# ag14774/MPILattice-Boltzmann

Measured on AMD Instinct MI355X. Metric: MLUPS, higher is better.
Workload: dtype f32; 1 GPU; synthetic 8192x8192 D2Q9-BGK deck (walls + p=0.005 random obstacles, splitmix64 seed 42), density 0.1 accel 0.005 omega 1.85; nx=8192, ny=8192, partitioning=single GPU, loop=single, macro_k=0, launches_per_exchange=1, step_allreduce=False, kernel=lbm_multi_kernel<4>

## Files before the change

mpilattice-boltzmann_amd/csrc/kernels/multi.h:

```cpp
#pragma once
#include "common.h"

namespace {

#if LBM_TILE_STAMPS
#define LBM_MSTAMP(i) do { if (blockIdx.x == (gridDim.x >> 1) && threadIdx.x == 0) g_tile_stamps[i] = __builtin_amdgcn_s_memtime(); } while (0)
#else
#define LBM_MSTAMP(i) do { } while (0)
#endif

template <int K, int GEOM = kGeomStd>
struct MultiGeom {
  static constexpr int TX = geom_tx(GEOM);
  static constexpr int TY = multi_ty(K, GEOM);
  static constexpr int LANES = multi_lanes(K, GEOM);
  static constexpr int EY = K - 1, EX = multi_ex(K - 1);
  static constexpr int W = TX + 2 * EX, H = TY + 2 * EY;
  static constexpr int cells = W * H;
  static constexpr size_t lds_bytes = sizeof(float) * 9 * cells + sizeof(double) * K * (LANES / 64) + (K >= 2 ? cells / 2 : 0);
  static constexpr int blocks_per_cu = lds_bytes * 8 <= 160 * 1024 ? 8 : static_cast<int>(160 * 1024 / lds_bytes);
  static constexpr int waves_per_simd = blocks_per_cu * (LANES / 64) / 4 < LBM_MWAVES ? (blocks_per_cu * (LANES / 64) / 4 < 1 ? 1 : blocks_per_cu * (LANES / 64) / 4) : LBM_MWAVES;
  static constexpr bool owned_lanes = K == 4 && GEOM == kGeomTall;
  static constexpr int ring_pairs(int j) { return 2 * (K - j) * (TX / 2 + multi_ex(K - j)) + TY * multi_ex(K - j); }
};

struct MultiArgs {
  const float* src;
  float* dst;
  const float* srck[9];
  float* dstk[9];
  const uint32_t* mask;
  size_t ps;
  int nx;
  int row_first, rows_compute;
  int rows_storage;
  int count_first, count_end;
  int y_periodic;
  int y0_global, ny_global;
// ... 46 lines not shown
constexpr uint32_t kPairObstacles = 3u,
                   kPairKept = 4u,
                   kPairAccelRow = 8u,
                   kPairComputed = 16u,
                   kPairCounted = 32u;
__device__ __forceinline__ uint32_t pair_flag_bits(uint32_t mbits, bool kept, bool accel_row, bool counted)
{
  return mbits | (kept ? kPairKept : 0u) | (accel_row ? kPairAccelRow : 0u) | kPairComputed | (counted ? kPairCounted : 0u);
}

template <int K, int TERMS, int GEOM, int PART>
__global__ void __launch_bounds__((MultiGeom<K, GEOM>::LANES), (MultiGeom<K, GEOM>::waves_per_simd)) lbm_multi_kernel(const MultiArgs a)
{
  using G = MultiGeom<K, GEOM>;
  constexpr int TX = G::TX, EX = G::EX, EY = G::EY, W = G::W, WH = G::W / 2, kCells = G::cells, kLanes = G::LANES, kWaves = kLanes / 64, TY = G::TY;
  extern __shared__ __attribute__((aligned(16))) float lds[];
  double* red = reinterpret_cast<double*>(lds + 9 * kCells);
  uint8_t* pair_flags = reinterpret_cast<uint8_t*>(red + K * kWaves);
  const int tid = threadIdx.x;

  if (blockIdx.x == 0) {
    constexpr int kReadyWords = PART == kPartTile ? 4 : PART == kPartReady ? 2 : 0;
    if constexpr (kReadyWords > 0) {
      if (a.ready_epoch != 0ull && tid == 0) {
#pragma unroll
        for (int d = 0; d < kReadyWords; ++d) __hip_atomic_store(d < 2 ? a.ready[d] : a.ready_x[d - 2], a.ready_epoch, __ATOMIC_RELAXED, __HIP_MEMORY_SCOPE_SYSTEM);
      }
    }
    for (int v = 0; v < a.n_prev_vecs; ++v) {
      double s = 0.0;
      for (int i = tid; i < a.n_prev; i += kLanes) s += a.prev_partials[static_cast<size_t>(v) * a.n_prev + i];
      s = wave_sum(s);
// ... 111 lines not shown
  };
  auto classify = [&](auto count_c, const int fx, const int fy, const bool own, bool& kept, bool& counted) __attribute__((always_inline)) {
    constexpr bool COUNT = decltype(count_c)::value;
    const int srow = sy0 + fy - EY, gxo = x0 + fx - EX;
    kept = own;
    if (!inner) kept = kept && gxo < nx && srow < a.row_first + a.rows_compute;
    counted = COUNT ? (kept && srow >= a.count_first && srow < a.count_end) : kept;
    if constexpr (XR && COUNT) {
      kept = kept && gxo >= a.keep_x0 && gxo < a.keep_x1;
      counted = counted && kept && gxo >= a.cx0 && gxo < a.cx1;
    }
  };
  auto read_pair = [&](const int rd, const int fx, const int fy, f2 (&p)[9]) __attribute__((always_inline)) {
    const int ci = fy * W + fx - rd;
    const int cs = fy * W + (fx >> 1) - rd;
    p[2] = *reinterpret_cast<const f2*>(lds + 2 * kCells + ci - W);
    p[4] = *reinterpret_cast<const f2*>(lds + 4 * kCells + ci + W);
    p[1] = f2{lds[1 * kCells + cs - 1], lds[1 * kCells + cs + WH]};
    p[5] = f2{lds[5 * kCells + cs - W - 1], lds[5 * kCells + cs - W + WH]};
    p[8] = f2{lds[8 * kCells + cs + W - 1], lds[8 * kCells + cs + W + WH]};
    p[3] = f2{lds[3 * kCells + cs], lds[3 * kCells + cs + WH + 1]};
    p[6] = f2{lds[6 * kCells + cs - W], lds[6 * kCells + cs - W + WH + 1]};
    p[7] = f2{lds[7 * kCells + cs + W], lds[7 * kCells + cs + W + WH + 1]};
  };
  auto kept_cell = [&](const int fx, const int fy) __attribute__((always_inline)) { return tile_row_base + __mul24(fy - EY, nx) + x0 + fx - EX; };

  auto k_substeps = [&](auto count_c) __attribute__((always_inline)) {
    constexpr bool COUNT = decltype(count_c)::value;
    {
      const int ey = ksteps - 1, ex = multi_ex(ey);
      const int wp = (TX + 2 * ex) / 2;
      const int np = wp * (TY + 2 * ey);
  #pragma unroll 1
      for (int i = tid; i < np; i += kLanes) {
        const int ry = i / wp, rp = i - ry * wp;
        const int fx = EX - ex + 2 * rp, fy = EY - ey + ry;
        f2 p[9], out[9];
        uint32_t mbits = 0, o_here = 0;
// ... 74 lines not shown
    constexpr bool COUNT = decltype(count_c)::value;
    constexpr int TP = TX / 2;
    static_assert(TP * TY == kLanes && G::ring_pairs(1) <= kLanes, "one owned pair and at most one ring pair per lane and sub-step");
    auto ring_pos = [&](auto jc, const int i, int& fx, int& fy) __attribute__((always_inline)) {
      constexpr int ey = K - decltype(jc)::value, ex = multi_ex(ey), ep = ex / 2, wp = TP + ep * 2, band = ey * wp;
      if (i < 2 * band) {
        const bool top = i >= band;
        const int q = top ? i - band : i, ry = q / wp, rp = q - ry * wp;
        fy = top ? EY + TY + ry : EY - ey + ry;
        fx = EX - ex + 2 * rp;
      } else {
        const int q = i - 2 * band, ry = q / (2 * ep), c = q - ry * (2 * ep);
        fy = EY + ry;
        fx = EX - ex + 2 * (c < ep ? c : c + TP);
      }
    };
    auto relax = [&](const f2 (&p)[9], const uint32_t mbits, const bool accel, const uint32_t skip, f2 (&out)[9]) __attribute__((always_inline)) {
      const double term = finish_pair<TERMS>(p, mbits, a.omega, false, false, a.accel_w1, a.accel_w2, skip, out);
      if (tile_accel) accelerate_pair(out, mbits, accel, a.accel_w1, a.accel_w2);
      return term;
    };
    const int py = tid / TP, ofx = EX + 2 * (tid - py * TP), ofy = EY + py;
    f2 own0 = f2{0.0f, 0.0f};
    uint32_t ofl = 0;
    if (!COUNT && inner) {
      const float* const here0 = a.srck[0], * const here1 = a.srck[1] - 1, * const here3 = a.srck[3] + 1;
      const float* const south2 = a.srck[2] - nx, * const south5 = a.srck[5] - 1 - nx, * const south6 = a.srck[6] + 1 - nx;
      const float* const north4 = a.srck[4] + nx, * const north8 = a.srck[8] - 1 + nx, * const north7 = a.srck[7] + 1 + nx;
      typedef const __attribute__((address_space(1))) char* global_bytes;
      const uint32_t* mask_arg = a.mask;
// ... 9 lines not shown
        p[5] = at_byte<f2u>(south5, o);
        p[8] = at_byte<f2u>(north8, o);
        p[3] = at_byte<f2u>(here3, o);
        p[6] = at_byte<f2u>(south6, o);
        p[7] = at_byte<f2u>(north7, o);
        mbits = (*(const __attribute__((address_space(1))) uint32_t*)(mask + 4u * (static_cast<uint32_t>(cell) >> 5)) >> (cell & 31)) & 3u;
        return o;
      };
      {
        f2 p[9], out[9];
        uint32_t mbits;
        pull_inner(ofx, ofy, p, mbits);
        const bool accel_row_here = on_accel_row(sy0 + py);
        acc[0] = relax(p, mbits, accel_row_here, mbits, out);
  #pragma unroll
        for (int k = 1; k < 9; ++k) store_pair<W>(lds + k * kCells, k, ofy * W, ofx, out[k]);
        own0 = out[0];
        ofl = pair_flag_bits(mbits, true, accel_row_here, false);
      }
      if (tid < G::ring_pairs(1)) {
        int fx, fy;
        ring_pos(std::integral_constant<int, 1>{}, tid, fx, fy);
        f2 p[9], out[9];
        uint32_t mbits;
        pull_inner(fx, fy, p, mbits);
        const bool accel_row_here = on_accel_row(sy0 + fy - EY);
        relax(p, mbits, accel_row_here, 3u, out);
  #pragma unroll
        for (int k = 0; k < 9; ++k) store_pair<W>(lds + k * kCells, k, fy * W, fx, out[k]);
        pair_flags[(fy * W + fx) >> 1] = static_cast<uint8_t>(pair_flag_bits(mbits, false, accel_row_here, false));
      }
    } else {
  #pragma unroll 1
    for (int item = 0; item < 2; ++item) {
      const bool own = item == 0;
      if (!own && tid >= G::ring_pairs(1)) break;
      int fx = ofx, fy = ofy;
      if (!own) ring_pos(std::integral_constant<int, 1>{}, tid, fx, fy);
      f2 p[9];
      uint32_t mbits = 0, fl = 0, o_here = 0;
      int sr = 0;
      if (pull(fx, fy, p, mbits, sr, o_here)) {
        bool kept, counted;
        classify(count_c, fx, fy, own, kept, counted);
        const bool accel_row_here = on_accel_row(sr);
        f2 out[9];
        const double term = relax(p, mbits, accel_row_here, counted ? mbits : 3u, out);
  #pragma unroll
        for (int k = 1; k < 9; ++k) store_pair<W>(lds + k * kCells, k, fy * W, fx, out[k]);
        fl = pair_flag_bits(mbits, kept, accel_row_here, COUNT && counted);
        if (own) {
          acc[0] = term;
          own0 = out[0];
        } else {
          store_pair<W>(lds, 0, fy * W, fx, out[0]);
        }
      }
      if (own) ofl = fl;
      else pair_flags[(fy * W + fx) >> 1] = static_cast<uint8_t>(fl);
    }
    }
    LBM_MSTAMP(1);
    __syncthreads();
    LBM_MSTAMP(2);
    auto in_lds_substep = [&](auto jc) __attribute__((always_inline)) {
      constexpr int j = decltype(jc)::value;
      constexpr bool last = j == K;
      constexpr int rd = (j - 2) * W, wr = (j - 1) * W;
      f2 p[9], outs[9];
      read_pair(rd, ofx, ofy, p);
      p[0] = own0;
      const uint32_t mbits = ofl & kPairObstacles;
      const bool counted = (ofl & (COUNT ? kPairCounted : kPairKept)) != 0u;
      acc[j - 1] = relax(p, mbits, (!last || a.accel_last) && (ofl & kPairAccelRow), counted ? mbits : 3u, outs);
      own0 = outs[0];
      if constexpr (!last) {
        f2 q[9];
        int rfx = 0, rfy = 0;
        uint32_t rfl = 0;
        const bool ring = tid < G::ring_pairs(j);
        if (ring) {
          ring_pos(jc, tid, rfx, rfy);
          rfl = pair_flags[(rfy * W + rfx) >> 1];
          read_pair(rd, rfx, rfy, q);
          q[0] = *reinterpret_cast<const f2*>(lds + rfy * W + rfx - rd);
        }
        __syncthreads();
        if (ofl & kPairComputed) {
  #pragma unroll
          for (int k = 1; k < 9; ++k) store_pair<W>(lds + k * kCells, k, ofy * W - wr, ofx, outs[k]);
        }
        if (ring) {
          f2 routs[9];
          relax(q, rfl & kPairObstacles, (rfl & kPairAccelRow) != 0u, 3u, routs);
          if (rfl & kPairComputed) {
  #pragma unroll
            for (int k = 0; k < 9; ++k) store_pair<W>(lds + k * kCells, k, rfy * W - wr, rfx, routs[k]);
          }
        }
        __syncthreads();
      } else if (ofl & kPairKept) {
        const uint32_t o = 4u * static_cast<uint32_t>(kept_cell(ofx, ofy));
  #pragma unroll
        for (int k = 0; k < 9; ++k) __builtin_nontemporal_store(outs[k], &at_byte<f2>(a.dstk[k], o));
      }
      LBM_MSTAMP(1 + j);
    };
    in_lds_substep(std::integral_constant<int, 2>{});
    if constexpr (K >= 3) in_lds_substep(std::integral_constant<int, K >= 3 ? 3 : 2>{});
    if constexpr (K >= 4) in_lds_substep(std::integral_constant<int, K >= 4 ? 4 : 2>{});
  };
  auto substeps = [&](auto count_c) __attribute__((always_inline)) {
    if constexpr (G::owned_lanes) owned_substeps(count_c);
    else k_substeps(count_c);
  };

  if constexpr (PART == kPartGhost) {
    if (sy0 >= a.count_first && sy0 + TY <= a.count_end) substeps(std::false_type{});
    else substeps(std::true_type{});
  } else if constexpr (PART == kPartTile) {
    if (sy0 >= a.count_first && sy0 + TY <= a.count_end && x0 >= a.cx0 && x0 + TX <= a.cx1) substeps(std::false_type{});
    else substeps(std::true_type{});
  } else {
    substeps(std::false_type{});
  }

  if constexpr ((TERMS & ~kTermsFused) == kTermsCompensated && !G::owned_lanes) {
#pragma unroll
    for (int i = 0; i < K; ++i) acc[i] += static_cast<double>(acc_lo[i]);
  }
  if constexpr (K == 1) {
    const double w = wave_sum(acc[0]);
    if ((tid & 63) == 0) red[tid >> 6] = w;
  } else {
    static_assert(K <= 4, "wave_sum_vec4 carries four steps");
    const double w = wave_sum_vec4(acc[0], acc[1], K > 2 ? acc[2] : 0.0, K > 3 ? acc[K > 3 ? 3 : 0] : 0.0);
    const int q = wave_sum_slot<4>(tid & 63);
    if ((tid & 15) == 0 && q < K) red[q * kWaves + (tid >> 6)] = w;
  }
  lds_barrier();
  if (tid < ksteps) {
    double t = 0.0;
    for (int w = 0; w < kWaves; ++w) t += red[tid * kWaves + w];
    a.partials_out[static_cast<size_t>(tid) * a.ntiles_total + tile] = t;
  }
  LBM_MSTAMP(2 + K);
}

}
```

mpilattice-boltzmann_amd/csrc/lbm_geometry.h:

```cpp
#pragma once

namespace {

constexpr int kBlock = 256;
constexpr int kCellsPerLane = 4;
constexpr int kHaloGuard = 4;

constexpr int kTermsDouble = 0, kTermsFloat = 1, kTermsCompensated = 2, kTermsFused = 4;

constexpr int kMaxTileSteps = 8;

constexpr int kFoldSlices = 64;

constexpr int kPairCells = 2;

constexpr bool tile64_geom_ok(int t, int h) { return (t == 8 || t == 16) && (h == 4 || h == 8); }
constexpr int tile64_region(int t, int h) { return t + 2 * h; }
constexpr int tile64_block(int t, int h) { return (t == 8 && h == 4) ? 256 : 512; }
constexpr int tile64_lds_bytes(int t, int h)
{
  return tile64_region(t, h) * tile64_region(t, h) * (2 * 9 * 8 + 1) + 8 * h * (tile64_block(t, h) / 64);
}
constexpr int kTile64Rows = 4 * 2;
constexpr int tile64_row(int t, int h, bool full) { return ((t == 8 ? 2 : 0) + (h == 4 ? 1 : 0)) * 2 + (full ? 1 : 0); }
// ... 3 lines not shown
#define LBM_MTY 16
#define LBM_MLANES 512
#endif
#ifndef LBM_MWAVES
#define LBM_MWAVES 6
#endif
#ifndef LBM_MTY4
#define LBM_MTY4 13
#endif
#ifndef LBM_MTY4T
#define LBM_MTY4T 24
#define LBM_MLANES4T 768
#endif
constexpr int kMTX = 64, kMTXNarrow = 32, kMTY = LBM_MTY, kMTY4 = LBM_MTY4, kMTY4Tall = LBM_MTY4T, kMLanes = LBM_MLANES, kMLanes4Tall = LBM_MLANES4T,
              kMaxMultiSteps = 4,
              kMaxGhost = 32,
              kMaxGroup = 8;
constexpr int kMinMultiTY = kMTY < kMTY4 ? (kMTY < kMTY4Tall ? kMTY : kMTY4Tall) : (kMTY4 < kMTY4Tall ? kMTY4 : kMTY4Tall);
constexpr int kGeomStd = 0, kGeomNarrow = 1, kGeomTall = 2;
constexpr int geom_tx(int g) { return g == kGeomNarrow ? kMTXNarrow : kMTX; }
constexpr int multi_ty(int k, int g) { return k >= 4 ? (g == kGeomTall ? kMTY4Tall : kMTY4) : kMTY; }
constexpr int multi_lanes(int k, int g) { return (k >= 4 && g == kGeomTall) ? kMLanes4Tall : kMLanes; }
constexpr int geom_for(int k, int g) { return (g == kGeomTall && k < 4) ? kGeomStd : g; }

constexpr int multi_ex(int ey) { return 2 * ((ey + 1) / 2); }

constexpr int kMulti64TX = 32, kMulti64TY = 16, kMulti64Lanes = 512, kMulti64MinK = 2, kMulti64MaxK = 4;
constexpr int kMulti64Accs = 4;
constexpr bool multi64_k_ok(int k) { return k >= kMulti64MinK && k <= kMulti64MaxK; }
constexpr int multi64_frame_x(int k) { return kMulti64TX + 2 * multi_ex(k - 1); }
constexpr int multi64_frame_y(int k) { return kMulti64TY + 2 * (k - 1); }
constexpr int multi64_lds_bytes(int k)
{
  return multi64_frame_x(k) * multi64_frame_y(k) * (9 * 8 + 1) + 8 * kMulti64Accs * (kMulti64Lanes / 64);
}
constexpr int kMulti64Rows = (kMulti64MaxK - kMulti64MinK + 1) * 2 * 2;
constexpr int multi64_row(int k, bool nt, bool full) { return ((k - kMulti64MinK) * 2 + (nt ? 1 : 0)) * 2 + (full ? 1 : 0); }
static_assert(kMulti64TX * kMulti64TY == kMulti64Lanes, "the last sub-step deals one owned cell to every lane");
static_assert(kMulti64MaxK <= kMulti64Accs, "one accumulator per sub-step");
static_assert((kMulti64TX + 2 * (kMulti64MaxK - 2)) * (kMulti64TY + 2 * (kMulti64MaxK - 2)) <= 2 * kMulti64Lanes, "a frame sub-step deals a lane at most two cells");
static_assert(multi64_lds_bytes(kMulti64MaxK) <= 160 * 1024, "a block's LDS: at most what a CU gives one workgroup");

constexpr int kPartPlain = 0, kPartGhost = 1, kPartReady = 2, kPartTile = 3;

constexpr int kMultiTermsFused = 3;
constexpr int kMultiTerms = 4, kMultiParts = 4, kMultiGeoms = 3, kMultiRowsPerGeom = kMaxMultiSteps * kMultiTerms * kMultiParts;
constexpr int multi_row(int k, int geom, int terms, int part) { return ((geom * kMaxMultiSteps + k - 1) * kMultiTerms + terms) * kMultiParts + part; }
constexpr int kTileTermsFused = 2, kTileTerms = 3, kTileRows = 4 * 2 * kTileTerms;
constexpr int tile_row(int t, int h, bool full, int terms) { return (((t == 8 ? 2 : 0) + (h == 4 ? 1 : 0)) * 2 + (full ? 1 : 0)) * kTileTerms + terms; }

}
```

mpilattice-boltzmann_amd/csrc/lbm_internal.h:

```cpp
#pragma once
#include <cstddef>
#include <string>

#include "lbm_d2q9.h"
#include "lbm_d2q9_f64.h"
#include "lbm_knobs.h"

namespace lbm_internal {
void set_error(const std::string& msg);

struct ContextPlan {
  int nx, y0, nyl;
  unsigned flags;
  int self_periodic, accel_row;
  int use_graph;
  float accel_w1, accel_w2, free_cells_inv;
  int multi_K;
  int ghost;
  int ghost_rows;
  int group_max;
  int ghost_x, x0, nxl, nx_global, tiles_px, tiles_py, tile_rx, tile_ry;
  long long ncells, ncells_storage, ps, grid_floats;
  int mask_words, nxp;
  int nt_stores, lane_cells;
// ... 92 lines not shown
struct MacroRows { int bottom_edge_rows, interior_rows, top_edge_rows, left_cols, right_cols; };
MacroRows macro_rows(const ContextPlan& plan, int k, int ext);
bool edge_rows_suffice(const ContextPlan& plan, const GroupPlan& g, const MacroRows& rows, int next_total);
struct ColumnMessagePlan { int per, blocks; };
ColumnMessagePlan plan_column_message(const ContextPlan& plan, int cols, int max_blocks, const long long* peer, int npeer);
}

extern "C" int lbm_plan_next(int K, int four_rows, int tail4, int left);
extern "C" int lbm_plan_group_for(int K, int four_rows, int tail4, int ghost, int group_max, int left, int* steps, int cap);
extern "C" int lbm_plan_group(int K, int ghost, int group_max, int left, int* steps, int cap);
extern "C" int lbm_plan_sizeof(void);
extern "C" int lbm_plan_whole(const lbm_params* p, int free_cells, int y0, int ny_local, unsigned flags, int has_global_map, lbm_internal::ContextPlan* out);
extern "C" int lbm_plan_rank(const lbm_params* p, int free_cells, int nranks, int rank, unsigned flags, lbm_internal::ContextPlan* out);
extern "C" int lbm_plan_tile(const lbm_params* p, int free_cells, int px, int py, int rank, unsigned flags, lbm_internal::ContextPlan* out);
extern "C" int lbm_plan_kernel_name(const lbm_internal::ContextPlan* plan, char* kernel_name, size_t len);
extern "C" int lbm_plan_launch_sizeof(void);
extern "C" int lbm_plan_launch(const lbm_internal::ContextPlan* plan, int k, int ext, int which, int says_ready, lbm_internal::LaunchPlan* out);
extern "C" int lbm_plan_run_launches(const lbm_internal::ContextPlan* plan, int n_steps, int schedule, lbm_internal::LaunchPlan* out, int cap);
extern "C" int lbm_plan_edge_rows_suffice(const lbm_internal::ContextPlan* plan, int left);
extern "C" int lbm_plan64_sizeof(void);
extern "C" int lbm_plan64_whole(const lbm64_params* p, unsigned flags, lbm_internal::Plan64* out);
extern "C" int lbm_plan64_kernel_name(const lbm_internal::Plan64* plan, char* kernel_name, size_t len);
extern "C" int lbm_plan64_run_launches(const lbm_internal::Plan64* plan, int n_steps, int* steps, int* full, int cap);
extern "C" int lbm_plan64_multi_sizeof(void);
extern "C" int lbm_plan64_multi(const lbm64_params* p, unsigned flags, lbm_internal::PlanMulti64* out);
extern "C" int lbm_plan64_multi_kernel_name(const lbm_internal::PlanMulti64* plan, char* kernel_name, size_t len);
extern "C" int lbm_plan64_multi_run_launches(const lbm_internal::PlanMulti64* plan, int n_steps, int* steps, int* full, int cap);
extern "C" int lbm_plan64_rows_sizeof(void);
extern "C" int lbm_plan64_rows(const lbm64_params* p, int nranks, int rank, unsigned flags, lbm_internal::PlanRows64* out);
extern "C" int lbm_plan64_rows_kernel_name(const lbm_internal::PlanRows64* plan, char* kernel_name, size_t len);
// ... 1 lines not shown
```

mpilattice-boltzmann_amd/csrc/lbm_kernels.hip:

```cpp

#include <hip/hip_runtime.h>

#include <algorithm>
#include <array>
#include <cstdint>
#include <cstdio>
#include <cstdlib>
#include <cstring>
#include <string>
#include <thread>
#include <type_traits>
#include <utility>
#include <vector>

#include "lbm_d2q9.h"
#include "lbm_internal.h"
#include "lbm_knobs.h"
#include "kernels/common.h"
#include "kernels/step.h"
#include "kernels/tile.h"
#include "kernels/multi.h"
#include "kernels/aux.h"
#include "kernels/p2p.h"

// ... 151 lines not shown
{
  kStepKernels[c->plan.lane_cells == 1][c->plan.nt_stores][c->plan.fused]<<<dim3(blocks + 1), dim3(kBlock), 0, s>>>(a);
}

struct MultiKernel { void (*fn)(MultiArgs); size_t lds_bytes; };
static_assert(kTermsDouble == 0 && kTermsFloat == 1 && kTermsCompensated == 2 && kPartPlain == 0 && kPartTile == 3 && kGeomTall == 2, "the values index the table");
template <int ROW>
constexpr MultiKernel multi_kernel_row()
{
  constexpr int PART = ROW % kMultiParts, TERMS = ROW / kMultiParts % kMultiTerms, K = ROW / (kMultiParts * kMultiTerms) % kMaxMultiSteps + 1,
                GEOM = geom_for(K, ROW / kMultiRowsPerGeom);
  static_assert(multi_row(K, ROW / kMultiRowsPerGeom, TERMS, PART) == ROW, "multi_row and its inverse");
  static_assert(MultiGeom<K, GEOM>::LANES == multi_lanes(K, ROW / kMultiRowsPerGeom), "LaunchPlan::lanes is the row's block size");
  return {&lbm_multi_kernel<K, TERMS == kMultiTermsFused ? (kTermsCompensated | kTermsFused) : TERMS, GEOM, PART>, MultiGeom<K, GEOM>::lds_bytes};
}
template <size_t... ROW>
constexpr std::array<MultiKernel, sizeof...(ROW)> multi_kernel_rows(std::index_sequence<ROW...>) { return {{multi_kernel_row<static_cast<int>(ROW)>()...}}; }
constexpr auto kMultiKernels = multi_kernel_rows(std::make_index_sequence<kMultiGeoms * kMultiRowsPerGeom>{});

template <typename Table>
hipError_t raise_lds_limits(const Table& rows, int first, int end)
{
  for (int r = first; r < end; ++r) {
    if (rows[r].lds_bytes <= 65536) continue;
    const hipError_t e = hipFuncSetAttribute(reinterpret_cast<const void*>(rows[r].fn), hipFuncAttributeMaxDynamicSharedMemorySize, static_cast<int>(rows[r].lds_bytes));
    if (e != hipSuccess) return e;
  }
  return hipSuccess;
}
hipError_t raise_multi_lds_limits_for(int geom)
{
  return raise_lds_limits(kMultiKernels, geom * kMultiRowsPerGeom, (geom + 1) * kMultiRowsPerGeom);
}

using lbm_internal::LaunchPlan;
using lbm_internal::GroupPlan;
using lbm_internal::kLaunchWhole;
using lbm_internal::kLaunchInterior;
using lbm_internal::kLaunchEdge;

void launch_multi(lbm_ctx* c, const LaunchPlan& l, bool accel_last, bool fold, hipStream_t s)
{
  MultiArgs a{};
  a.src = c->grid[c->cur]; a.dst = c->grid[c->cur ^ 1];
  for (int k = 0; k < 9; ++k) { a.srck[k] = a.src + k * c->plan.ps; a.dstk[k] = a.dst + k * c->plan.ps; }
  a.mask = c->mask; a.ps = c->plan.ps; a.nx = c->p.nx;
  a.row_first = l.row_first; a.rows_compute = l.rows_compute; a.rows_storage = l.rows_storage;
// ... 245 lines not shown
  return 0;
}

static ColWindow col_window(const lbm_ctx* c) { return ColWindow{static_cast<unsigned>(c->p.nx), static_cast<unsigned>(c->plan.ghost_x), static_cast<unsigned>(c->plan.nxl)}; }
static size_t owned_cells(const lbm_ctx* c) { return static_cast<size_t>(c->plan.nxl) * c->plan.nyl; }

extern "C" {

int lbm_create(lbm_ctx** out, const lbm_params* p, int free_cells, const int* obstacles_rows, int y0,
               int ny_local, int device, unsigned flags)
{
  if (!out || !p || !obstacles_rows) { lbm_internal::set_error("lbm_create: null argument"); return 1; }
  *out = nullptr;
  const Knobs knobs = knobs_from_env();
  lbm_internal::ContextPlan plan;
  const int status = lbm_internal::plan_whole(knobs, p, free_cells, y0, ny_local, flags, false, &plan);
  return create_impl(out, status, plan, knobs, p, free_cells, obstacles_rows, nullptr, nullptr, device);
}

int lbm_create_global(lbm_ctx** out, const lbm_params* p, int free_cells, const int* obstacles_all, int y0,
                      int ny_local, int device, unsigned flags)
{
  if (!obstacles_all || !p || y0 < 0) { lbm_internal::set_error("lbm_create_global: bad argument"); return 1; }
  if (!out) { lbm_internal::set_error("lbm_create: null argument"); return 1; }
  *out = nullptr;
  const Knobs knobs = knobs_from_env();
  lbm_internal::ContextPlan plan;
  const int status = lbm_internal::plan_whole(knobs, p, free_cells, y0, ny_local, flags, true, &plan);
  return create_impl(out, status, plan, knobs, p, free_cells, obstacles_all + static_cast<size_t>(y0) * p->nx, obstacles_all, nullptr, device);
}

int lbm_create_rank(lbm_ctx** out, const lbm_params* p, int free_cells, const int* obstacle_window, int nranks,
                    int rank, int device, unsigned flags)
{
  if (!obstacle_window) { lbm_internal::set_error("lbm_create_rank: null argument"); return 1; }
  if (!out) {
    lbm_layout lay;
    if (lbm_rank_layout(p, nranks, rank, flags, &lay) == 0) lbm_internal::set_error("lbm_create: null argument");
    return 1;
  }
  *out = nullptr;
  const Knobs knobs = knobs_from_env();
  lbm_internal::ContextPlan plan;
// ... 591 lines not shown
```

mpilattice-boltzmann_amd/csrc/lbm_knobs.h:

```cpp
#pragma once

#include <climits>
#include <cstdlib>
#include <cstring>

constexpr int kKnobUnset = INT_MIN;
constexpr int kScheduleSerial = 0, kScheduleEdge = 1;

inline int schedule_of(const char* v) { return !std::strcmp(v, "serial") ? kScheduleSerial : !std::strcmp(v, "edge") ? kScheduleEdge : kKnobUnset; }
inline int knob_or(int v, int fallback) { return v == kKnobUnset ? fallback : v; }

#define LBM_KNOBS(X)                                                                        \
                                            \
  X(LBM_TUNE_SKEW,              skew,              24,         std::atoi)                   \
  X(LBM_TUNE_MAXBLOCKS,         maxblocks,         16384,      std::atoi)                   \
  X(LBM_TUNE_NARROW_MAX,        narrow_max,        65536,      std::atoi)                   \
  X(LBM_TUNE_TILE_MAX,          tile_max,          131072,     std::atoi)                   \
  X(LBM_TUNE_TILE_GEOM,         tile_geom,         kKnobUnset, std::atoi)                   \
  X(LBM_TUNE_TILE_SINGLE_MAX,   tile_single_max,   512,        std::atoi)                   \
  X(LBM_TUNE_TILE64_MAX,        tile64_max,        1 << 20,    std::atoi)                   \
  X(LBM_TUNE_TILE64_GEOM,       tile64_geom,       kKnobUnset, std::atoi)                   \
  X(LBM_TUNE_MULTI64_K,         multi64_k,         kKnobUnset, std::atoi)                   \
  X(LBM_TUNE_MULTI64_MIN,       multi64_min,       1 << 20,    std::atoi)                   \
  X(LBM_TUNE_MULTI_K,           multi_k,           kKnobUnset, std::atoi)                   \
  X(LBM_TUNE_MULTI_TAIL4,       multi_tail4,       1,          std::atoi)                   \
  X(LBM_TUNE_MULTI_TILE,        multi_tile,        kKnobUnset, std::atoi)                   \
  X(LBM_TUNE_NARROW_TILE_MAX,   narrow_tile_max,   1 << 17,    std::atoi)                   \
  X(LBM_TUNE_TALL_TILE_MIN,     tall_tile_min,     1 << 20,    std::atoi)                   \
  X(LBM_TUNE_MULTI_GEOM,        multi_geom,        -1,         std::atoi)                   \
  X(LBM_TUNE_MULTI_REMAP,       multi_remap,       1,          std::atoi)                   \
  X(LBM_TUNE_TILE_PAD_GRID,     tile_pad_grid,     1,          std::atoi)                   \
  X(LBM_TUNE_TERMS,             terms,             -1,         std::atoi)                   \
  X(LBM_TUNE_FOLD_SLICED_MIN,   fold_sliced_min,   1024,       std::atoi)                   \
  X(LBM_TUNE_OBS_CHUNK_CELLS,   obs_chunk_cells,   16 << 20,   std::atoi)                   \
  X(LBM_DEBUG_ADDR,             debug_addr,        0,          std::atoi)                   \
                    \
  X(LBM_TUNE_MACRO_K,           macro_k,           4,          std::atoi)                   \
  X(LBM_TUNE_MACRO_GHOST,       macro_ghost,       kKnobUnset, std::atoi)                   \
  X(LBM_TUNE_MACRO_GROUP,       macro_group,       kKnobUnset, std::atoi)                   \
// ... 27 lines not shown
```

mpilattice-boltzmann_amd/csrc/lbm_plan.cpp:

```cpp

#include <algorithm>
#include <cstdio>
#include <cstring>
#include <vector>

#include "lbm_d2q9.h"
#include "lbm_geometry.h"
#include "lbm_internal.h"
#include "lbm_knobs.h"

using lbm_internal::ContextPlan;
using lbm_internal::set_error;

namespace lbm_internal {

size_t plane_stride_floats(size_t ncells, int skew)
{
  size_t s = (ncells + 64 + 63) / 64 * 64;
  if ((s / 64) % 2 == 0) s += 64;
  if (ncells >= (1u << 20)) s += 64 * static_cast<size_t>(skew);
  return s;
}

int pick_iters(long long quads, int max_blocks)
// ... 112 lines not shown
  out->ghost_y = (py == 1 && !knobs.tile_ghost_rows) ? 0 : ghost;
  return 0;
}

struct TileSpec { int px, py, rx, ry, x0, nxl, ghost_x, nx_global, ghost_rows; };

void plan_multi(const Knobs& knobs, bool tile_rank, ContextPlan& c)
{
  c.multi_geom = pick_geom(knobs, static_cast<size_t>(c.ncells));
  if (tile_rank && c.ghost_rows == 0 && c.multi_geom == kGeomTall && knobs.multi_geom < 0) {
    auto over = [&](int ty) { return static_cast<double>((c.nyl + ty - 1) / ty * ty) / c.nyl; };
    if (over(kMTY4Tall) - over(kMTY4) > 0.03) c.multi_geom = kGeomStd;
  }
  c.multi_tx = geom_tx(c.multi_geom);
  c.multi_tiles_x = (c.nx + c.multi_tx - 1) / c.multi_tx;
  if (c.multi_K > 0) c.partials_cap = std::max(c.partials_cap, kMaxMultiSteps * c.multi_tiles_x * ((c.nyl + 2 * c.ghost_rows + kMinMultiTY - 1) / kMinMultiTY) + 1);
}

int plan_context(const Knobs& knobs, const lbm_params* p, int free_cells, bool has_global_map, bool has_window, int forced_k, int forced_ghost,
                 int y0, int ny_local, unsigned flags, const TileSpec* tile, ContextPlan* out)
{
  if (!p || !out) { set_error("lbm_create: null argument"); return lbm_internal::kPlanRefused; }
  if (p->nx < 1) { set_error("lbm_create: nx must be positive"); return lbm_internal::kPlanRefused; }
  if (p->ny < 3) { set_error("lbm_create: ny must be >= 3 (accelerate_flow works on row ny-2, d2q9-bgk.c:449)"); return lbm_internal::kPlanRefused; }
  if (ny_local < 1 || y0 < 0 || y0 + ny_local > p->ny) { set_error("lbm_create: partition rows out of range"); return lbm_internal::kPlanRefused; }
  if (free_cells <= 0) { set_error("lbm_create: free_cells must be positive"); return lbm_internal::kPlanRefused; }
  if (flags & LBM_FLAG_FUSED_ARITH) {
    if (flags & (LBM_FLAG_FAST_AVVELS | LBM_FLAG_EXACT_AVVELS)) {
      set_error("lbm_create: LBM_FLAG_FUSED_ARITH cannot be combined with LBM_FLAG_FAST_AVVELS or LBM_FLAG_EXACT_AVVELS (the fused kernels carry each family's default sum|u| terms only)");
      return lbm_internal::kPlanRefused;
    }
// ... 78 lines not shown
    c.tile_T = geom / 10; c.tile_H = geom % 10;
    if (!((c.tile_T == 16 || c.tile_T == 8) && (c.tile_H == 8 || c.tile_H == 4))) { c.tile_T = 16; c.tile_H = 4; }
  }
  c.tile_single_max = knobs.tile_single_max;
  c.n_tiles = (p->nx % c.tile_T == 0 && ny_local % c.tile_T == 0) ? (p->nx / c.tile_T) * (ny_local / c.tile_T) : 0;
  c.tile_kernel = self_periodic && c.n_tiles > 0 &&
                  ncells <= static_cast<size_t>(knobs.tile_max);
  c.multi_geom = kGeomStd; c.multi_tx = kMTX;
  if (c.ghost > 0) {
    c.pack_floats = c.ghost_rows > 0 ? 9LL * c.ghost * p->nx : 0;
    c.pack_alloc_floats = 2LL * 9 * std::max(c.ghost_rows, 1) * p->nx;
    c.pack_floats_x = c.ghost_x > 0 ? 9LL * ny_local * c.ghost_x : 0;
    c.tile_kernel = 0;
    plan_multi(knobs, tile != nullptr, c);
  } else if (!c.tile_kernel && self_periodic && whole_grid_tiled(p->nx, ny_local)) {
    c.multi_K = std::min(std::max(knob_or(knobs.multi_k, ncells >= size_t(768) * 768 ? 4 : 3), 0), kMaxMultiSteps);
    plan_multi(knobs, false, c);
  } else if (c.tile_kernel) {
    c.partials_cap = std::max(c.partials_cap, kMaxTileSteps * c.n_tiles + 1);
  }
  *out = c;
  return lbm_internal::kPlanOk;
}

}

namespace lbm_internal {

int plan_whole(const Knobs& knobs, const lbm_params* p, int free_cells, int y0, int ny_local, unsigned flags, bool has_global_map, ContextPlan* out)
{
  return plan_context(knobs, p, free_cells, has_global_map, false, has_global_map ? -1 : 0, 0, y0, ny_local, flags, nullptr, out);
// ... 237 lines not shown
    else { a.tile_count = r.bottom_edge_rows * a.tiles_x; a.tile_begin2 = (r.bottom_edge_rows + r.interior_rows) * a.tiles_x; a.tile_count2 = r.top_edge_rows * a.tiles_x; }
  }
  int blocks = a.tile_count + a.tile_count2;
  for (int i = 0; i < a.nrect; ++i) blocks += a.rect[i].count;
  a.xcd_remap = (knobs.multi_remap && blocks % 8 == 0 && blocks >= 64) ? 1 : 0;
  a.nblocks = blocks;
  if (c.ghost_x > 0 && knobs.multi_remap && blocks >= 64 && blocks % 8 != 0 && knobs.tile_pad_grid) {
    blocks = (blocks + 7) / 8 * 8;
    a.xcd_remap = 1;
  }
  a.launched_blocks = blocks;
  a.part = c.ghost_x > 0 ? kPartTile : ext > 0 ? kPartGhost : says_ready ? kPartReady : kPartPlain;
  const int steps = std::min(k, static_cast<int>(kMaxMultiSteps));
  a.row = multi_row(steps, c.multi_geom, c.fused ? kMultiTermsFused : c.multi_terms, a.part);
  a.lanes = multi_lanes(steps, c.multi_geom);
  *out = a;
}

void plan_tile_launch(const ContextPlan& c, int left, LaunchPlan* out)
{
  LaunchPlan a{};
  a.k = std::min(c.tile_H, left);
  a.full = a.k == c.tile_H;
  a.tiles_x = c.nx / c.tile_T;
  a.ntiles_total = a.tile_count = a.nblocks = a.launched_blocks = c.n_tiles;
  a.row = tile_row(c.tile_T, c.tile_H, a.full != 0, c.fused ? kTileTermsFused : c.fast_avvels ? kTermsFloat : kTermsDouble);
  *out = a;
}

bool edge_rows_suffice(const ContextPlan& c, const GroupPlan& g, const MacroRows& rows, int next_total)
// ... 12 lines not shown
  const int per = all_mult(4) ? 4 : all_mult(2) ? 2 : 1;
  const long long work = 18LL * c.nyl * (cols / per);
  return {per, static_cast<int>(std::max(1LL, std::min(static_cast<long long>(max_blocks), (work + 1023) / 1024)))};
}

}

extern "C" {

int lbm_plan_next(int K, int four_rows, int tail4, int left)
{
  int k = left < K ? left : K;
  if (!four_rows || !tail4) return k;
  if (K == 3 && ((left % 3 == 1 && left >= 4) || (left % 3 == 2 && left >= 8))) k = 4;
  if (K == 4 && ((left % 4 == 3) || (left % 4 == 2 && left >= 6) || (left % 4 == 1 && left >= 9))) k = 3;
  return k;
}

int lbm_plan_group_for(int K, int four_rows, int tail4, int ghost, int group_max, int left, int* steps, int cap)
{
  int n = 0, used = 0;
  while (left > 0 && n < group_max) {
    const int k = lbm_plan_next(K, four_rows, tail4, left);
    if (n > 0 && used + k > ghost) break;
    if (n < cap) steps[n] = k;
    ++n; used += k; left -= k;
  }
  return n;
}

// ... 58 lines not shown
int lbm_plan_rank(const lbm_params* p, int free_cells, int nranks, int rank, unsigned flags, ContextPlan* out)
{
  return lbm_internal::plan_rank(knobs_from_env(), p, free_cells, nranks, rank, flags, out) ? 1 : 0;
}
int lbm_plan_tile(const lbm_params* p, int free_cells, int px, int py, int rank, unsigned flags, ContextPlan* out)
{
  return lbm_internal::plan_tile(knobs_from_env(), p, free_cells, px, py, rank, flags, out) ? 1 : 0;
}
int lbm_plan_kernel_name(const ContextPlan* plan, char* kernel_name, size_t len)
{
  if (!plan || !kernel_name || !len) { set_error("lbm_plan_kernel_name: null argument"); return 1; }
  lbm_internal::plan_kernel_name(*plan, kernel_name, len);
  return 0;
}

int lbm_plan_launch_sizeof(void) { return static_cast<int>(sizeof(lbm_internal::LaunchPlan)); }
int lbm_plan_launch(const ContextPlan* plan, int k, int ext, int which, int says_ready, lbm_internal::LaunchPlan* out)
{
  if (!plan || !out || plan->multi_tiles_x <= 0 || k < 1 || k > kMaxMultiSteps || ext < 0 || ext > kMaxGhost || which < lbm_internal::kLaunchWhole || which > lbm_internal::kLaunchEdge) {
    set_error("lbm_plan_launch: bad argument");
    return 1;
  }
  lbm_internal::plan_launch(*plan, knobs_from_env(), k, ext, which, says_ready != 0, out);
  return 0;
}

int lbm_plan_run_launches(const ContextPlan* plan, int n_steps, int schedule, lbm_internal::LaunchPlan* out, int cap)
{
  using namespace lbm_internal;
  if (!plan || n_steps < 0 || cap < 0 || (cap > 0 && !out) || (schedule != kScheduleSerial && schedule != kScheduleEdge)) { set_error("lbm_plan_run_launches: bad argument"); return -1; }
  const Knobs knobs = knobs_from_env();
  const KernelFamily family = family_of(*plan);
  int n = 0;
  LaunchPlan l;
// ... 102 lines not shown
```

Before: 268,000 MLUPS.

## Add five-step temporally blocked whole-grid kernel with compact population-0 LDS storage

Adds a K=5 variant of the multi-step in-LDS kernel for the tall tile geometry, chosen for large self-periodic whole grids. Each launch then advances five time steps per global read and write of the lattice. To fit the larger frame in LDS, population 0 is kept in registers for owned pairs and in a small ring buffer for halo pairs instead of a full plane. The cost is more halo recompute, lower occupancy (two blocks per CU), and a runtime occupancy check that falls back to four steps.

After: 273,600 MLUPS, median of 6. +2.1%, better.

```diff
diff --git a/mpilattice-boltzmann_amd/csrc/kernels/multi.h b/mpilattice-boltzmann_amd/csrc/kernels/multi.h
--- a/mpilattice-boltzmann_amd/csrc/kernels/multi.h
+++ b/mpilattice-boltzmann_amd/csrc/kernels/multi.h
@@ -17,11 +17,16 @@
   static constexpr int EY = K - 1, EX = multi_ex(K - 1);
   static constexpr int W = TX + 2 * EX, H = TY + 2 * EY;
   static constexpr int cells = W * H;
-  static constexpr size_t lds_bytes = sizeof(float) * 9 * cells + sizeof(double) * K * (LANES / 64) + (K >= 2 ? cells / 2 : 0);
+  static constexpr bool compact0 = multi_compact0(K, GEOM);
+  static constexpr int planes = compact0 ? 8 : 9, first_plane = compact0 ? 1 : 0;
+  static constexpr int ring0_floats = compact0 ? 2 * multi_ring_pairs(K, GEOM, 1) : 0;
+  static constexpr size_t lds_bytes = multi_lds_bytes(K, GEOM);
+  static_assert(lds_bytes == sizeof(float) * (planes * cells + ring0_floats) + sizeof(double) * K * (LANES / 64) + (K >= 2 ? cells / 2 : 0), "the kernel's layout and lbm_geometry.h agree");
+  static_assert(W == multi_frame_w(K, GEOM) && H == multi_frame_h(K, GEOM), "the frame of lbm_geometry.h");
   static constexpr int blocks_per_cu = lds_bytes * 8 <= 160 * 1024 ? 8 : static_cast<int>(160 * 1024 / lds_bytes);
   static constexpr int waves_per_simd = blocks_per_cu * (LANES / 64) / 4 < LBM_MWAVES ? (blocks_per_cu * (LANES / 64) / 4 < 1 ? 1 : blocks_per_cu * (LANES / 64) / 4) : LBM_MWAVES;
-  static constexpr bool owned_lanes = K == 4 && GEOM == kGeomTall;
-  static constexpr int ring_pairs(int j) { return 2 * (K - j) * (TX / 2 + multi_ex(K - j)) + TY * multi_ex(K - j); }
+  static constexpr bool owned_lanes = K >= 4 && GEOM == kGeomTall;
+  static constexpr int ring_pairs(int j) { return multi_ring_pairs(K, GEOM, j); }
 };
 
 struct MultiArgs {
@@ -98,8 +103,9 @@
 {
   using G = MultiGeom<K, GEOM>;
   constexpr int TX = G::TX, EX = G::EX, EY = G::EY, W = G::W, WH = G::W / 2, kCells = G::cells, kLanes = G::LANES, kWaves = kLanes / 64, TY = G::TY;
+  constexpr int kPlanes = G::planes, kPl = G::first_plane;
   extern __shared__ __attribute__((aligned(16))) float lds[];
-  double* red = reinterpret_cast<double*>(lds + 9 * kCells);
+  double* red = reinterpret_cast<double*>(lds + kPlanes * kCells + G::ring0_floats);
   uint8_t* pair_flags = reinterpret_cast<uint8_t*>(red + K * kWaves);
   const int tid = threadIdx.x;
 
@@ -241,14 +247,14 @@
   auto read_pair = [&](const int rd, const int fx, const int fy, f2 (&p)[9]) __attribute__((always_inline)) {
     const int ci = fy * W + fx - rd;
     const int cs = fy * W + (fx >> 1) - rd;
-    p[2] = *reinterpret_cast<const f2*>(lds + 2 * kCells + ci - W);
-    p[4] = *reinterpret_cast<const f2*>(lds + 4 * kCells + ci + W);
-    p[1] = f2{lds[1 * kCells + cs - 1], lds[1 * kCells + cs + WH]};
-    p[5] = f2{lds[5 * kCells + cs - W - 1], lds[5 * kCells + cs - W + WH]};
-    p[8] = f2{lds[8 * kCells + cs + W - 1], lds[8 * kCells + cs + W + WH]};
-    p[3] = f2{lds[3 * kCells + cs], lds[3 * kCells + cs + WH + 1]};
-    p[6] = f2{lds[6 * kCells + cs - W], lds[6 * kCells + cs - W + WH + 1]};
-    p[7] = f2{lds[7 * kCells + cs + W], lds[7 * kCells + cs + W + WH + 1]};
+    p[2] = *reinterpret_cast<const f2*>(lds + (2 - kPl) * kCells + ci - W);
+    p[4] = *reinterpret_cast<const f2*>(lds + (4 - kPl) * kCells + ci + W);
+    p[1] = f2{lds[(1 - kPl) * kCells + cs - 1], lds[(1 - kPl) * kCells + cs + WH]};
+    p[5] = f2{lds[(5 - kPl) * kCells + cs - W - 1], lds[(5 - kPl) * kCells + cs - W + WH]};
+    p[8] = f2{lds[(8 - kPl) * kCells + cs + W - 1], lds[(8 - kPl) * kCells + cs + W + WH]};
+    p[3] = f2{lds[(3 - kPl) * kCells + cs], lds[(3 - kPl) * kCells + cs + WH + 1]};
+    p[6] = f2{lds[(6 - kPl) * kCells + cs - W], lds[(6 - kPl) * kCells + cs - W + WH + 1]};
+    p[7] = f2{lds[(7 - kPl) * kCells + cs + W], lds[(7 - kPl) * kCells + cs + W + WH + 1]};
   };
   auto kept_cell = [&](const int fx, const int fy) __attribute__((always_inline)) { return tile_row_base + __mul24(fy - EY, nx) + x0 + fx - EX; };
 
@@ -353,6 +359,13 @@
         fy = EY + ry;
         fx = EX - ex + 2 * (c < ep ? c : c + TP);
       }
+    };
+    [[maybe_unused]] f2* const ring0 = reinterpret_cast<f2*>(lds + kPlanes * kCells);
+    [[maybe_unused]] auto ring0_at = [&](const int fx, const int fy) __attribute__((always_inline)) -> f2* {
+      constexpr int ep = EX / 2, wp = TP + ep * 2, band = EY * wp;
+      const int rp = fx >> 1;
+      const int i = fy < EY ? fy * wp + rp : fy >= EY + TY ? band + (fy - EY - TY) * wp + rp : 2 * band + (fy - EY) * (2 * ep) + (rp < ep ? rp : rp - TP);
+      return ring0 + i;
     };
     auto relax = [&](const f2 (&p)[9], const uint32_t mbits, const bool accel, const uint32_t skip, f2 (&out)[9]) __attribute__((always_inline)) {
       const double term = finish_pair<TERMS>(p, mbits, a.omega, false, false, a.accel_w1, a.accel_w2, skip, out);
@@ -392,7 +405,7 @@
         const bool accel_row_here = on_accel_row(sy0 + py);
         acc[0] = relax(p, mbits, accel_row_here, mbits, out);
   #pragma unroll
-        for (int k = 1; k < 9; ++k) store_pair<W>(lds + k * kCells, k, ofy * W, ofx, out[k]);
+        for (int k = 1; k < 9; ++k) store_pair<W>(lds + (k - kPl) * kCells, k, ofy * W, ofx, out[k]);
         own0 = out[0];
         ofl = pair_flag_bits(mbits, true, accel_row_here, false);
       }
@@ -405,7 +418,8 @@
         const bool accel_row_here = on_accel_row(sy0 + fy - EY);
         relax(p, mbits, accel_row_here, 3u, out);
   #pragma unroll
-        for (int k = 0; k < 9; ++k) store_pair<W>(lds + k * kCells, k, fy * W, fx, out[k]);
+        for (int k = kPl; k < 9; ++k) store_pair<W>(lds + (k - kPl) * kCells, k, fy * W, fx, out[k]);
+        if constexpr (G::compact0) ring0[tid] = out[0];
         pair_flags[(fy * W + fx) >> 1] = static_cast<uint8_t>(pair_flag_bits(mbits, false, accel_row_here, false));
       }
     } else {
@@ -425,11 +439,13 @@
         f2 out[9];
         const double term = relax(p, mbits, accel_row_here, counted ? mbits : 3u, out);
   #pragma unroll
-        for (int k = 1; k < 9; ++k) store_pair<W>(lds + k * kCells, k, fy * W, fx, out[k]);
+        for (int k = 1; k < 9; ++k) store_pair<W>(lds + (k - kPl) * kCells, k, fy * W, fx, out[k]);
         fl = pair_flag_bits(mbits, kept, accel_row_here, COUNT && counted);
         if (own) {
           acc[0] = term;
           own0 = out[0];
+        } else if constexpr (G::compact0) {
+          ring0[tid] = out[0];
         } else {
           store_pair<W>(lds, 0, fy * W, fx, out[0]);
         }
@@ -456,24 +472,27 @@
         f2 q[9];
         int rfx = 0, rfy = 0;
         uint32_t rfl = 0;
+        [[maybe_unused]] f2* r0 = nullptr;
         const bool ring = tid < G::ring_pairs(j);
         if (ring) {
           ring_pos(jc, tid, rfx, rfy);
           rfl = pair_flags[(rfy * W + rfx) >> 1];
           read_pair(rd, rfx, rfy, q);
-          q[0] = *reinterpret_cast<const f2*>(lds + rfy * W + rfx - rd);
+          if constexpr (G::compact0) { r0 = ring0_at(rfx, rfy); q[0] = *r0; }
+          else q[0] = *reinterpret_cast<const f2*>(lds + rfy * W + rfx - rd);
         }
         __syncthreads();
         if (ofl & kPairComputed) {
   #pragma unroll
-          for (int k = 1; k < 9; ++k) store_pair<W>(lds + k * kCells, k, ofy * W - wr, ofx, outs[k]);
+          for (int k = 1; k < 9; ++k) store_pair<W>(lds + (k - kPl) * kCells, k, ofy * W - wr, ofx, outs[k]);
         }
         if (ring) {
           f2 routs[9];
           relax(q, rfl & kPairObstacles, (rfl & kPairAccelRow) != 0u, 3u, routs);
           if (rfl & kPairComputed) {
   #pragma unroll
-            for (int k = 0; k < 9; ++k) store_pair<W>(lds + k * kCells, k, rfy * W - wr, rfx, routs[k]);
+            for (int k = kPl; k < 9; ++k) store_pair<W>(lds + (k - kPl) * kCells, k, rfy * W - wr, rfx, routs[k]);
+            if constexpr (G::compact0) *r0 = routs[0];
           }
         }
         __syncthreads();
@@ -487,6 +506,7 @@
     in_lds_substep(std::integral_constant<int, 2>{});
     if constexpr (K >= 3) in_lds_substep(std::integral_constant<int, K >= 3 ? 3 : 2>{});
     if constexpr (K >= 4) in_lds_substep(std::integral_constant<int, K >= 4 ? 4 : 2>{});
+    if constexpr (K >= 5) in_lds_substep(std::integral_constant<int, K >= 5 ? 5 : 2>{});
   };
   auto substeps = [&](auto count_c) __attribute__((always_inline)) {
     if constexpr (G::owned_lanes) owned_substeps(count_c);
@@ -510,11 +530,18 @@
   if constexpr (K == 1) {
     const double w = wave_sum(acc[0]);
     if ((tid & 63) == 0) red[tid >> 6] = w;
-  } else {
-    static_assert(K <= 4, "wave_sum_vec4 carries four steps");
+  } else if constexpr (K <= 4) {
     const double w = wave_sum_vec4(acc[0], acc[1], K > 2 ? acc[2] : 0.0, K > 3 ? acc[K > 3 ? 3 : 0] : 0.0);
     const int q = wave_sum_slot<4>(tid & 63);
     if ((tid & 15) == 0 && q < K) red[q * kWaves + (tid >> 6)] = w;
+  } else {
+    static_assert(K <= 8, "wave_sum_vec8 carries eight steps");
+    double acc8[8];
+#pragma unroll
+    for (int i = 0; i < 8; ++i) acc8[i] = i < K ? acc[i < K ? i : 0] : 0.0;
+    const double w = wave_sum_vec8(acc8);
+    const int q = wave_sum_slot<8>(tid & 63);
+    if ((tid & 7) == 0 && q < K) red[q * kWaves + (tid >> 6)] = w;
   }
   lds_barrier();
   if (tid < ksteps) {
diff --git a/mpilattice-boltzmann_amd/csrc/lbm_geometry.h b/mpilattice-boltzmann_amd/csrc/lbm_geometry.h
--- a/mpilattice-boltzmann_amd/csrc/lbm_geometry.h
+++ b/mpilattice-boltzmann_amd/csrc/lbm_geometry.h
@@ -41,6 +41,7 @@
 #endif
 constexpr int kMTX = 64, kMTXNarrow = 32, kMTY = LBM_MTY, kMTY4 = LBM_MTY4, kMTY4Tall = LBM_MTY4T, kMLanes = LBM_MLANES, kMLanes4Tall = LBM_MLANES4T,
               kMaxMultiSteps = 4,
+              kMaxWholeGridSteps = 5,
               kMaxGhost = 32,
               kMaxGroup = 8;
 constexpr int kMinMultiTY = kMTY < kMTY4 ? (kMTY < kMTY4Tall ? kMTY : kMTY4Tall) : (kMTY4 < kMTY4Tall ? kMTY4 : kMTY4Tall);
@@ -51,6 +52,17 @@
 constexpr int geom_for(int k, int g) { return (g == kGeomTall && k < 4) ? kGeomStd : g; }
 
 constexpr int multi_ex(int ey) { return 2 * ((ey + 1) / 2); }
+
+constexpr bool multi_compact0(int k, int g) { return k == kMaxWholeGridSteps && g == kGeomTall; }
+constexpr int multi_frame_w(int k, int g) { return geom_tx(g) + 2 * multi_ex(k - 1); }
+constexpr int multi_frame_h(int k, int g) { return multi_ty(k, g) + 2 * (k - 1); }
+constexpr int multi_ring_pairs(int k, int g, int j) { return 2 * (k - j) * (geom_tx(g) / 2 + multi_ex(k - j)) + multi_ty(k, g) * multi_ex(k - j); }
+constexpr int multi_lds_bytes(int k, int g)
+{
+  const int cells = multi_frame_w(k, g) * multi_frame_h(k, g);
+  return 4 * (multi_compact0(k, g) ? 8 : 9) * cells + (multi_compact0(k, g) ? 8 * multi_ring_pairs(k, g, 1) : 0) + 8 * k * (multi_lanes(k, g) / 64) + (k >= 2 ? cells / 2 : 0);
+}
+static_assert(multi_lds_bytes(kMaxWholeGridSteps, kGeomTall) * 2 <= 160 * 1024, "two blocks of the five-step launch per CU");
 
 constexpr int kMulti64TX = 32, kMulti64TY = 16, kMulti64Lanes = 512, kMulti64MinK = 2, kMulti64MaxK = 4;
 constexpr int kMulti64Accs = 4;
@@ -73,6 +85,8 @@
 constexpr int kMultiTermsFused = 3;
 constexpr int kMultiTerms = 4, kMultiParts = 4, kMultiGeoms = 3, kMultiRowsPerGeom = kMaxMultiSteps * kMultiTerms * kMultiParts;
 constexpr int multi_row(int k, int geom, int terms, int part) { return ((geom * kMaxMultiSteps + k - 1) * kMultiTerms + terms) * kMultiParts + part; }
+constexpr int kMultiRows = kMultiGeoms * kMultiRowsPerGeom, kMultiRowsTotal = kMultiRows + kMultiTerms;
+constexpr int multi_row5(int terms) { return kMultiRows + terms; }
 constexpr int kTileTermsFused = 2, kTileTerms = 3, kTileRows = 4 * 2 * kTileTerms;
 constexpr int tile_row(int t, int h, bool full, int terms) { return (((t == 8 ? 2 : 0) + (h == 4 ? 1 : 0)) * 2 + (full ? 1 : 0)) * kTileTerms + terms; }
 
diff --git a/mpilattice-boltzmann_amd/csrc/lbm_internal.h b/mpilattice-boltzmann_amd/csrc/lbm_internal.h
--- a/mpilattice-boltzmann_amd/csrc/lbm_internal.h
+++ b/mpilattice-boltzmann_amd/csrc/lbm_internal.h
@@ -130,6 +130,7 @@
 extern "C" int lbm_plan_rank(const lbm_params* p, int free_cells, int nranks, int rank, unsigned flags, lbm_internal::ContextPlan* out);
 extern "C" int lbm_plan_tile(const lbm_params* p, int free_cells, int px, int py, int rank, unsigned flags, lbm_internal::ContextPlan* out);
 extern "C" int lbm_plan_kernel_name(const lbm_internal::ContextPlan* plan, char* kernel_name, size_t len);
+extern "C" int lbm_plan_multi_lds_bytes(int k, int geom);
 extern "C" int lbm_plan_launch_sizeof(void);
 extern "C" int lbm_plan_launch(const lbm_internal::ContextPlan* plan, int k, int ext, int which, int says_ready, lbm_internal::LaunchPlan* out);
 extern "C" int lbm_plan_run_launches(const lbm_internal::ContextPlan* plan, int n_steps, int schedule, lbm_internal::LaunchPlan* out, int cap);
diff --git a/mpilattice-boltzmann_amd/csrc/lbm_kernels.hip b/mpilattice-boltzmann_amd/csrc/lbm_kernels.hip
--- a/mpilattice-boltzmann_amd/csrc/lbm_kernels.hip
+++ b/mpilattice-boltzmann_amd/csrc/lbm_kernels.hip
@@ -189,9 +189,21 @@
   static_assert(MultiGeom<K, GEOM>::LANES == multi_lanes(K, ROW / kMultiRowsPerGeom), "LaunchPlan::lanes is the row's block size");
   return {&lbm_multi_kernel<K, TERMS == kMultiTermsFused ? (kTermsCompensated | kTermsFused) : TERMS, GEOM, PART>, MultiGeom<K, GEOM>::lds_bytes};
 }
+template <int TERMS>
+constexpr MultiKernel multi_kernel_row5()
+{
+  using G = MultiGeom<kMaxWholeGridSteps, kGeomTall>;
+  static_assert(G::LANES == multi_lanes(kMaxWholeGridSteps, kGeomTall) && G::owned_lanes && G::compact0, "the tall tile, one owned pair per lane, population 0 out of the frame");
+  return {&lbm_multi_kernel<kMaxWholeGridSteps, TERMS == kMultiTermsFused ? (kTermsCompensated | kTermsFused) : TERMS, kGeomTall, kPartPlain>, G::lds_bytes};
+}
 template <size_t... ROW>
-constexpr std::array<MultiKernel, sizeof...(ROW)> multi_kernel_rows(std::index_sequence<ROW...>) { return {{multi_kernel_row<static_cast<int>(ROW)>()...}}; }
-constexpr auto kMultiKernels = multi_kernel_rows(std::make_index_sequence<kMultiGeoms * kMultiRowsPerGeom>{});
+constexpr std::array<MultiKernel, sizeof...(ROW) + kMultiTerms> multi_kernel_rows(std::index_sequence<ROW...>)
+{
+  static_assert(kMultiTerms == 4 && multi_row5(3) == sizeof...(ROW) + 3, "the four rows below");
+  return {{multi_kernel_row<static_cast<int>(ROW)>()..., multi_kernel_row5<0>(), multi_kernel_row5<1>(), multi_kernel_row5<2>(), multi_kernel_row5<3>()}};
+}
+constexpr auto kMultiKernels = multi_kernel_rows(std::make_index_sequence<kMultiRows>{});
+static_assert(kMultiKernels.size() == kMultiRowsTotal, "every row a LaunchPlan can name");
 
 template <typename Table>
 hipError_t raise_lds_limits(const Table& rows, int first, int end)
@@ -205,7 +217,30 @@
 }
 hipError_t raise_multi_lds_limits_for(int geom)
 {
-  return raise_lds_limits(kMultiKernels, geom * kMultiRowsPerGeom, (geom + 1) * kMultiRowsPerGeom);
+  const hipError_t e = raise_lds_limits(kMultiKernels, geom * kMultiRowsPerGeom, (geom + 1) * kMultiRowsPerGeom);
+  if (e != hipSuccess || geom != kGeomTall) return e;
+  return raise_lds_limits(kMultiKernels, kMultiRows, kMultiRowsTotal);
+}
+
+bool five_step_launch_fits(int terms_row)
+{
+  const MultiKernel& k = kMultiKernels[multi_row5(terms_row)];
+  if (hipFuncSetAttribute(reinterpret_cast<const void*>(k.fn), hipFuncAttributeMaxDynamicSharedMemorySize, static_cast<int>(k.lds_bytes)) != hipSuccess) { (void)hipGetLastError(); return false; }
+  int blocks = 0;
+  if (hipOccupancyMaxActiveBlocksPerMultiprocessor(&blocks, reinterpret_cast<const void*>(k.fn), multi_lanes(kMaxWholeGridSteps, kGeomTall), k.lds_bytes) != hipSuccess) { (void)hipGetLastError(); return false; }
+  return blocks >= 2;
+}
+
+int plan_whole_on_device(const Knobs& knobs, const lbm_params* p, int free_cells, int y0, int ny_local, unsigned flags, bool has_global_map, int device,
+                         lbm_internal::ContextPlan* plan)
+{
+  const int status = lbm_internal::plan_whole(knobs, p, free_cells, y0, ny_local, flags, has_global_map, plan);
+  if (status != lbm_internal::kPlanOk || plan->multi_K != kMaxWholeGridSteps) return status;
+  if (hipSetDevice(device) != hipSuccess) { (void)hipGetLastError(); return status; }
+  if (five_step_launch_fits(plan->fused ? kMultiTermsFused : plan->multi_terms)) return status;
+  Knobs four = knobs;
+  four.multi_k = kMaxMultiSteps;
+  return lbm_internal::plan_whole(four, p, free_cells, y0, ny_local, flags, has_global_map, plan);
 }
 
 using lbm_internal::LaunchPlan;
@@ -481,7 +516,7 @@
   *out = nullptr;
   const Knobs knobs = knobs_from_env();
   lbm_internal::ContextPlan plan;
-  const int status = lbm_internal::plan_whole(knobs, p, free_cells, y0, ny_local, flags, false, &plan);
+  const int status = plan_whole_on_device(knobs, p, free_cells, y0, ny_local, flags, false, device, &plan);
   return create_impl(out, status, plan, knobs, p, free_cells, obstacles_rows, nullptr, nullptr, device);
 }
 
@@ -493,7 +528,7 @@
   *out = nullptr;
   const Knobs knobs = knobs_from_env();
   lbm_internal::ContextPlan plan;
-  const int status = lbm_internal::plan_whole(knobs, p, free_cells, y0, ny_local, flags, true, &plan);
+  const int status = plan_whole_on_device(knobs, p, free_cells, y0, ny_local, flags, true, device, &plan);
   return create_impl(out, status, plan, knobs, p, free_cells, obstacles_all + static_cast<size_t>(y0) * p->nx, obstacles_all, nullptr, device);
 }
 
diff --git a/mpilattice-boltzmann_amd/csrc/lbm_knobs.h b/mpilattice-boltzmann_amd/csrc/lbm_knobs.h
--- a/mpilattice-boltzmann_amd/csrc/lbm_knobs.h
+++ b/mpilattice-boltzmann_amd/csrc/lbm_knobs.h
@@ -23,6 +23,7 @@
   X(LBM_TUNE_MULTI64_K,         multi64_k,         kKnobUnset, std::atoi)                   \
   X(LBM_TUNE_MULTI64_MIN,       multi64_min,       1 << 20,    std::atoi)                   \
   X(LBM_TUNE_MULTI_K,           multi_k,           kKnobUnset, std::atoi)                   \
+  X(LBM_TUNE_MULTI5_MIN,        multi5_min,        1 << 26,    std::atoi)                   \
   X(LBM_TUNE_MULTI_TAIL4,       multi_tail4,       1,          std::atoi)                   \
   X(LBM_TUNE_MULTI_TILE,        multi_tile,        kKnobUnset, std::atoi)                   \
   X(LBM_TUNE_NARROW_TILE_MAX,   narrow_tile_max,   1 << 17,    std::atoi)                   \
diff --git a/mpilattice-boltzmann_amd/csrc/lbm_plan.cpp b/mpilattice-boltzmann_amd/csrc/lbm_plan.cpp
--- a/mpilattice-boltzmann_amd/csrc/lbm_plan.cpp
+++ b/mpilattice-boltzmann_amd/csrc/lbm_plan.cpp
@@ -150,7 +150,13 @@
   }
   c.multi_tx = geom_tx(c.multi_geom);
   c.multi_tiles_x = (c.nx + c.multi_tx - 1) / c.multi_tx;
-  if (c.multi_K > 0) c.partials_cap = std::max(c.partials_cap, kMaxMultiSteps * c.multi_tiles_x * ((c.nyl + 2 * c.ghost_rows + kMinMultiTY - 1) / kMinMultiTY) + 1);
+  const int vecs = c.multi_K > kMaxMultiSteps ? c.multi_K : kMaxMultiSteps;
+  if (c.multi_K > 0) c.partials_cap = std::max(c.partials_cap, vecs * c.multi_tiles_x * ((c.nyl + 2 * c.ghost_rows + kMinMultiTY - 1) / kMinMultiTY) + 1);
+}
+
+bool five_steps_eligible(const ContextPlan& c, unsigned flags)
+{
+  return c.self_periodic && c.ghost == 0 && c.ghost_x == 0 && !c.tile_kernel && !(flags & LBM_FLAG_ONE_STEP) && c.multi_geom == kGeomTall;
 }
 
 int plan_context(const Knobs& knobs, const lbm_params* p, int free_cells, bool has_global_map, bool has_window, int forced_k, int forced_ghost,
@@ -259,7 +265,10 @@
     c.tile_kernel = 0;
     plan_multi(knobs, tile != nullptr, c);
   } else if (!c.tile_kernel && self_periodic && whole_grid_tiled(p->nx, ny_local)) {
-    c.multi_K = std::min(std::max(knob_or(knobs.multi_k, ncells >= size_t(768) * 768 ? 4 : 3), 0), kMaxMultiSteps);
+    c.multi_geom = pick_geom(knobs, ncells);
+    const bool five_ok = five_steps_eligible(c, flags);
+    const int by_size = (five_ok && knobs.multi5_min > 0 && ncells >= static_cast<size_t>(knobs.multi5_min)) ? kMaxWholeGridSteps : ncells >= size_t(768) * 768 ? 4 : 3;
+    c.multi_K = std::min(std::max(knob_or(knobs.multi_k, by_size), 0), five_ok ? kMaxWholeGridSteps : kMaxMultiSteps);
     plan_multi(knobs, false, c);
   } else if (c.tile_kernel) {
     c.partials_cap = std::max(c.partials_cap, kMaxTileSteps * c.n_tiles + 1);
@@ -527,6 +536,10 @@
   const int steps = std::min(k, static_cast<int>(kMaxMultiSteps));
   a.row = multi_row(steps, c.multi_geom, c.fused ? kMultiTermsFused : c.multi_terms, a.part);
   a.lanes = multi_lanes(steps, c.multi_geom);
+  if (k == kMaxWholeGridSteps && c.multi_K == kMaxWholeGridSteps) {
+    a.row = multi_row5(c.fused ? kMultiTermsFused : c.multi_terms);
+    a.lanes = multi_lanes(k, c.multi_geom);
+  }
   *out = a;
 }
 
@@ -569,6 +582,7 @@
   if (!four_rows || !tail4) return k;
   if (K == 3 && ((left % 3 == 1 && left >= 4) || (left % 3 == 2 && left >= 8))) k = 4;
   if (K == 4 && ((left % 4 == 3) || (left % 4 == 2 && left >= 6) || (left % 4 == 1 && left >= 9))) k = 3;
+  if (K == 5 && left >= 3) k = (left == 5 || left >= 8) ? 5 : left == 7 ? 4 : left == 6 ? 3 : left;
   return k;
 }
 
@@ -657,10 +671,16 @@
   return 0;
 }
 
+int lbm_plan_multi_lds_bytes(int k, int geom)
+{
+  if (geom < kGeomStd || geom > kGeomTall || k < 1 || k > (geom == kGeomTall ? kMaxWholeGridSteps : kMaxMultiSteps)) return -1;
+  return multi_lds_bytes(k, geom_for(k, geom));
+}
+
 int lbm_plan_launch_sizeof(void) { return static_cast<int>(sizeof(lbm_internal::LaunchPlan)); }
 int lbm_plan_launch(const ContextPlan* plan, int k, int ext, int which, int says_ready, lbm_internal::LaunchPlan* out)
 {
-  if (!plan || !out || plan->multi_tiles_x <= 0 || k < 1 || k > kMaxMultiSteps || ext < 0 || ext > kMaxGhost || which < lbm_internal::kLaunchWhole || which > lbm_internal::kLaunchEdge) {
+  if (!plan || !out || plan->multi_tiles_x <= 0 || k < 1 || k > (plan->multi_K == kMaxWholeGridSteps ? kMaxWholeGridSteps : kMaxMultiSteps) || ext < 0 || ext > kMaxGhost || which < lbm_internal::kLaunchWhole || which > lbm_internal::kLaunchEdge) {
     set_error("lbm_plan_launch: bad argument");
     return 1;
   }
```
